# zser092/Focused-Attention-ViT

Measured on AMD Instinct MI355X. Metric: images/sec (train fwd+bwd) ViT-MHLA 224/p16, higher is better.
Workload: dtype bf16; 1 GPU; ViT-MHLA-Small (D384/12L/6H, window 7) 224x224 patch16, 197 tokens, 256 images/GPU; step = fwd + cross-entropy + bwd + grad all-reduce + AdamW; global_batch=256, parallelism=dp1, weights=random-init (seed 1234), hip_graph=False

## Files before the change

focused-attention-vit_amd/_abi.py:

```python
from __future__ import annotations

import ctypes as C
import os
import re

_HERE = os.path.dirname(os.path.abspath(__file__))
LIB_PATH = os.path.join(_HERE, "lib", "libfavit.so")
HEADER_PATH = os.path.join(os.path.dirname(_HERE), "include", "favit.h")

F32, BF16, FP8 = 0, 1, 2
F32X3 = 3
E4M3, E5M2 = 0, 1
ACT_NONE, ACT_GELU, ACT_DGELU, ACT_GELU_SAVEGRAD, ACT_MULAUX = 0, 1, 2, 3, 4
ERR_INVALID, ERR_UNSUPPORTED, ERR_ALIGN, ERR_LAUNCH = -1, -2, -3, -4
POOL = {"mean": 0, "max": 1, "attention": 2}

vp, i32, i64, u64, f32 = C.c_void_p, C.c_int32, C.c_int64, C.c_uint64, C.c_float


class GemmDesc(C.Structure):
    _fields_ = [
        ("A", vp), ("B", vp), ("C", vp), ("bias", vp), ("aux_in", vp), ("aux_out", vp), ("residual", vp),
        ("a_rowsum", vp),
        ("M", i64), ("N", i64), ("K", i64),
# ... 5 lines not shown
        ("scale_a", vp), ("scale_b", vp),
    ]


class SdpaDesc(C.Structure):
    _fields_ = [
        ("q", vp), ("k", vp), ("v", vp), ("o", vp), ("lse", vp), ("dout", vp), ("dq", vp), ("dk", vp), ("dv", vp),
        ("delta", vp), ("mask", vp), ("m_sb", i64), ("m_sq", i64),
        ("q_str", i64 * 3), ("k_str", i64 * 3), ("v_str", i64 * 3), ("o_str", i64 * 3), ("do_str", i64 * 3),
        ("dq_str", i64 * 3), ("dk_str", i64 * 3), ("dv_str", i64 * 3),
        ("B", i32), ("H", i32), ("Lq", i32), ("Lk", i32), ("hd", i32), ("dtype", i32),
        ("scale", f32), ("dropout_p", f32), ("seed", u64),
    ]


_SIGS = {
    "favit_abi_version": ([], C.c_int),
    "favit_strerror": ([C.c_int], C.c_char_p),
    "favit_set_dropout_epoch": ([vp], C.c_int),
    "favit_set_health_word": ([vp], C.c_int),
    "favit_gemm": ([C.POINTER(GemmDesc), vp], C.c_int),
    "favit_gemm_last_kernel": ([], C.c_char_p),
    "favit_ln_gemm": ([C.POINTER(GemmDesc), vp, i64, vp, vp, f32, vp, vp, vp, vp], C.c_int),
    "favit_gemm_grouped_tn": ([C.POINTER(GemmDesc), i32, vp], C.c_int),
    "favit_gemm_grouped_tn_workspace": ([C.POINTER(GemmDesc), i32], C.c_int64),
    "favit_gemm_grouped_tn_ws": ([C.POINTER(GemmDesc), i32, vp, i64, vp], C.c_int),
    "favit_gemm_grouped_last_splits": ([], C.c_int),
    "favit_cast": ([vp, C.c_int, vp, C.c_int, i64, vp], C.c_int),
    "favit_fp8_amax": ([vp, C.c_int, i64, i64, i64, vp, vp], C.c_int),
    "favit_fp8_quantize": ([vp, C.c_int, i64, i64, i64, vp, i64, vp, i64, C.c_int, vp, vp, vp, vp, vp, vp], C.c_int),
# ... 14 lines not shown
    "favit_mhla_attn_fwd": ([vp, vp, vp, i32, i32, i32, i32, i32, C.c_int, f32, u64, vp], C.c_int),
    "favit_mhla_attn_bwd": ([vp, vp, vp, vp, i32, i32, i32, i32, i32, C.c_int, f32, u64, vp], C.c_int),
    "favit_mhla_attn_lse_supported": ([i32, i32, i32, C.c_int], C.c_int),
    "favit_mhla_attn_fwd_lse": ([vp, vp, vp, vp, i32, i32, i32, i32, i32, C.c_int, f32, u64, vp], C.c_int),
    "favit_mhla_attn_bwd_lse": ([vp, vp, vp, vp, vp, vp, i32, i32, i32, i32, i32, C.c_int, f32, u64, vp], C.c_int),
    "favit_sdpa_fwd": ([C.POINTER(SdpaDesc), vp], C.c_int),
    "favit_sdpa_bwd": ([C.POINTER(SdpaDesc), vp], C.c_int),
    "favit_softmax_fwd": ([vp, vp, vp, C.c_int, vp, i64, i64, i32, i64, i32, i32, f32, u64, vp], C.c_int),
    "favit_softmax_bwd": ([vp, C.c_int, vp, vp, C.c_int, i64, i32, i32, f32, u64, vp], C.c_int),
    "favit_patchify_fwd": ([vp, vp, C.c_int, i32, i32, i32, i32, vp], C.c_int),
    "favit_patchify_bwd": ([vp, vp, i32, i32, i32, i32, vp], C.c_int),
    "favit_embed_prologue_fwd": ([vp, vp, vp, vp, i32, i32, i32, vp], C.c_int),
    "favit_embed_prologue_bwd": ([vp, vp, C.c_int, vp, vp, i32, i32, i32, vp], C.c_int),
    "favit_rows_cut_fwd": ([vp, vp, i32, i32, i32, i32, i32, vp], C.c_int),
    "favit_rows_cut_bwd": ([vp, vp, vp, C.c_int, i32, i32, i32, i32, i32, vp], C.c_int),
    "favit_dropout": ([vp, vp, C.c_int, i64, f32, u64, vp], C.c_int),
    "favit_sppp_map_patches": ([vp, vp, vp, vp, vp, vp, i32, i32, i32, vp], C.c_int),
    "favit_sppp_pool_fwd": ([vp, vp, vp, vp, vp, i32, i32, i32, i32, i32, vp], C.c_int),
    "favit_sppp_pool_bwd": ([vp, vp, vp, vp, vp, vp, vp, i32, i32, i32, i32, i32, vp], C.c_int),
    "favit_sppp_centroids": ([vp, vp, i32, i32, i32, vp], C.c_int),
    "favit_sppp_posenc_fwd": ([vp, vp, vp, i32, i32, i32, i32, vp], C.c_int),
    "favit_image_transform": ([vp, vp, vp, vp, vp, i32, i32, i32, i32, i32, i32, C.POINTER(f32), C.POINTER(f32), vp], C.c_int),
    "favit_image_transform_ragged": ([vp, vp, vp, vp, vp, vp, i32, i32, i32, i32, C.POINTER(f32), C.POINTER(f32), vp], C.c_int),
    "favit_slic_features_workspace": ([i32, i32, i32], C.c_int64),
    "favit_slic_features": ([vp, vp, i32, i32, i32, f32, i32, vp, vp], C.c_int),
    "favit_slic_cluster_workspace": ([i32, i32], C.c_int64),
    "favit_slic_cluster": ([vp, vp, vp, i32, i32, i32, i32, i32, i64, i32, vp, vp], C.c_int),
    "favit_slic_connect": ([vp, vp, vp, vp, vp, i32, i32, i32, i32, vp], C.c_int),
    "favit_cross_entropy": ([vp, vp, vp, vp, i32, i32, f32, vp], C.c_int),
    "favit_adamw": ([vp, vp, vp, vp, vp, i64, f32, f32, f32, f32, f32, f32, f32, f32, vp], C.c_int),
# ... 49 lines not shown
```

focused-attention-vit_amd/functional.py:

```python
from __future__ import annotations

import os
import weakref
from typing import List, Optional, Sequence, Tuple

import torch

from . import kernels as K
from ._abi import ACT_DGELU, ACT_GELU, ACT_GELU_SAVEGRAD, ACT_MULAUX, ACT_NONE

_STATE = {"cdt": torch.float32, "epoch": 0, "direct_grads": True, "grad_ready": None}


def set_direct_grads(on: bool) -> None:
    _STATE["direct_grads"] = bool(on)


def set_grad_ready_hook(fn) -> None:
    _STATE["grad_ready"] = fn


def _gt(p):
    if p is None or not _STATE["direct_grads"] or not getattr(p, "requires_grad", False):
        return None
# ... 546 lines not shown
        wp_c = wcast(wp)
        y = lin_fwd(o, wp_c, bp.detach(), M, D, D, torch.float32, residual=residual, drop=(pp, sp), site=wp)
        return y, (xn, weff, qkv, o, wp_c, mask, B, L, pa, sa, pp, sp, prm, lse)

    @staticmethod
    def out_dropout(saved):
        return saved[10], saved[11]

    def bwd(self, saved, dy_lp, premasked=False):
        xn, weff, qkv, o, wp_c, mask, B, L, pa, sa, pp, sp, prm, lse = saved
        wqkv, bqkv, wl, bl, wp, bp = prm
        M, D = xn.shape
        H, hd = self.H, D // self.H
        dym = K.dropout(dy_lp, pp, sp) if (pp > 0 and not premasked) else dy_lp
        do = lin_bwd_x(dym, wp_c, M, D, D, xn.dtype, site=wp)
        dwp, dbp = lin_bwd_w(dym, o, M, D, D, wp=wp, bp=bp)
        dqkv = K.mhla_attn_bwd(qkv, do, B, L, H, hd, self.W, mask, pa, sa, o=o if lse is not None else None, lse=lse)
        dxn = lin_bwd_x(dqkv, weff, M, 3 * D, D, xn.dtype, site=wqkv)
        dweff, dbeff = lin_bwd_w(dqkv, xn, M, 3 * D, D)
        tg = [_gt(p) for p in (wqkv, bqkv, wl, bl)]
        if all(t is not None for t in tg) and _DEFER["on"]:
            _DEFER["fold"].append((dweff, dbeff, wqkv.detach(), bqkv.detach(), wl.detach(), tg, H, (wqkv, bqkv, wl, bl)))
            return dxn, [None, None, None, None, dwp, dbp]
        if (_DEFER["on"] and not wqkv.requires_grad and not bqkv.requires_grad and tg[2] is not None and tg[3] is not None):
            _DEFER["fold"].append((dweff, dbeff, wqkv.detach(), bqkv.detach(), wl.detach(), [None, None, tg[2], tg[3]], H,
                                   (wl, bl)))
            return dxn, [None, None, None, None, dwp, dbp]
        flush_wgrads()
        if all(t is not None for t in tg):
            with _side_stream(dweff, dbeff):
                K.mhla_fold_bwd(dweff, dbeff, wqkv, bqkv, wl, H, out=tg)
                _ready(wqkv, bqkv, wl, bl)
            return dxn, [None, None, None, None, dwp, dbp]
        join_side_stream()
        dwqkv, dbqkv, dwl, dbl = K.mhla_fold_bwd(dweff, dbeff, wqkv, bqkv, wl, H)
        return dxn, [dwqkv, dbqkv, dwl, dbl, dwp, dbp]


class DenseChain:
    q8_fwd, q8_bwd = 0, 2
    """vit.MultiHeadAttention.forward (models/vit.py:77-104) and, with the
    nn.MultiheadAttention parameter names, the use_mhla=False branch
    (models/vit_mhla.py:57-62,96-101).  mask: key-keep [B,L] (torch MHA) or None."""

    def __init__(self, H, p_attn=0.0, p_proj=0.0, torch_mha=False):
        self.H, self.p_attn, self.p_proj, self.torch_mha = H, p_attn, p_proj, torch_mha
        self.names = (("in_proj_weight", "in_proj_bias", "out_proj.weight", "out_proj.bias") if torch_mha
                      else ("qkv.weight", "qkv.bias", "proj.weight", "proj.bias"))

    def _views(self, t, B, L, D, hd):
        ld = 3 * D
# ... 103 lines not shown
    def fwd(self, xn, prm, residual, training, ln=None):
        w1, b1, w2, b2 = prm
        M, D = xn.shape if ln is None else ln[0].shape
        Hd = w1.shape[0]
        Do = w2.shape[0]
        p = self.p if training else 0.0
        s1 = _seed() if p > 0 else 0
        s2 = _seed() if p > 0 else 0
        w1_c, w2_c = wcast(w1), wcast(w2)
        if ln is not None:
            sg = True
            h, pre, xn, mu, rs = lin_fwd_ln(ln[:3], w1_c, b1.detach(), M, Hd, D, get_compute_dtype(), act=ACT_GELU_SAVEGRAD,
                                            want_pre=True, drop=(p, s1))
            ln[3][:] = [xn, mu, rs]
        else:
            sg = xn.dtype != torch.float32
            h, pre = lin_fwd(xn, w1_c, b1.detach(), M, Hd, D, xn.dtype, act=ACT_GELU_SAVEGRAD if sg else ACT_GELU,
                             want_pre=True, drop=(p, s1), site=w1)
        y = lin_fwd(h, w2_c, b2.detach(), M, Do, Hd, torch.float32, residual=residual, drop=(p, s2), site=w2)
        return y, (xn, (pre, sg), h, w1_c, w2_c, p, s1, s2, prm)

    @staticmethod
    def out_dropout(saved):
        return saved[5], saved[7]

    def bwd(self, saved, dy_lp, premasked=False):
        xn, (pre, sg), h, w1_c, w2_c, p, s1, s2, prm = saved
        w1, b1, w2, b2 = prm
        M, D = xn.shape
        Hd, Do = w1_c.shape[0], w2_c.shape[0]
        dym = K.dropout(dy_lp, p, s2) if (p > 0 and not premasked) else dy_lp
        dpre = lin_bwd_x(dym, w2_c, M, Do, Hd, xn.dtype, dgelu_pre=pre, pre_is_grad=sg, drop=(p, s1), site=w2)
        dw2, db2 = lin_bwd_w(dym, h, M, Do, Hd, wp=w2, bp=b2)
        dxn = lin_bwd_x(dpre, w1_c, M, Hd, D, xn.dtype, site=w1)
        dw1, db1 = lin_bwd_w(dpre, xn, M, Hd, D, wp=w1, bp=b1)
        return dxn, [dw1, db1, dw2, db2]


class OpFn(torch.autograd.Function):

    @staticmethod
    def forward(ctx, op, n_in, *tensors):
        K.require_gpu(*[t for t in tensors if t is not None])
        ins, prm = tensors[:n_in], tensors[n_in:]
        out, saved = op.fwd(ins, prm)
        ctx.op, ctx.saved, ctx.n_in, ctx.n_prm = op, saved, n_in, len(prm)
        return out

    @staticmethod
    def backward(ctx, dout):
        din, dprm = ctx.op.bwd(ctx.saved, _as_f32(dout), ctx.needs_input_grad[2:2 + ctx.n_in])
# ... 122 lines not shown


def cls_only_cuts(specs: Sequence["BlockSpec"], L: int, mask, training: bool):
    if os.environ.get("FAVIT_NO_PRUNE") or mask is not None or not specs or _STATE.get("fp8"):
        return None
    if not all(isinstance(s.attn, MHLAChain) and isinstance(s.mlp, MLPChain) for s in specs):
        return None
    if len({s.attn.W for s in specs}) != 1:
        return None
    if training and any(s.attn.p_attn > 0 or s.attn.p_proj > 0 or s.mlp.p > 0 for s in specs):
        return None
    plan = cls_plan(L, specs[0].attn.W, len(specs))
    return plan if any(c is not None for c in plan) else None


class EncoderOp:

    def __init__(self, blocks: List[BlockSpec], mask=None, training=False, cuts=None):
        self.blocks, self.mask, self.training = blocks, mask, training
        self.cuts = list(cuts) if cuts is not None else None
        if self.cuts is not None and (len(self.cuts) != len(blocks) or mask is not None):
            raise ValueError("cuts: one entry per block, and no attention mask")

    def fwd(self, ins, prm):
        (x,) = ins
        B, L, D = x.shape
        M = B * L
        L_in = L
        cdt = get_compute_dtype()
        x = _as_f32(x).reshape(M, D)
        tapes = []
        fuse_ok = _LN_FUSE and cdt == torch.bfloat16 and get_compute_mode() == "bf16" and D % 64 == 0 and D <= 512
        pre = [None] * len(self.blocks)
        idx, fp, off = [], [], 0
        for bi, bs in enumerate(self.blocks):
            if isinstance(bs.attn, MHLAChain):
                idx.append(bi)
                fp.append(tuple(prm[off + 2:off + 6]))
            off += bs.n
        if 2 <= len(idx) <= 32 and len({(self.blocks[i].attn.H, tuple(q[0].shape)) for i, q in zip(idx, fp)}) == 1:
            for bi, we in zip(idx, K.mhla_fold_fwd_multi(fp, self.blocks[idx[0]].attn.H, cdt)):
                pre[bi] = we
        off = 0
        for bi, bs in enumerate(self.blocks):
            p = list(prm[off:off + bs.n])
            off += bs.n
            na = len(bs.attn.names)
            g1, b1 = p[0], p[1]
            pa = p[2:2 + na]
            g2, b2 = p[2 + na], p[3 + na]
            pm = p[4 + na:]
            cut = None
            if self.cuts is not None and self.cuts[bi] is not None and sum(self.cuts[bi]) < L:
                ca, cb = self.cuts[bi]
                x = K.rows_cut_fwd(x, B, L, ca, cb, D).reshape(B * (ca + cb), D)
                cut = (L, ca, cb)
                L = ca + cb
                M = B * L
            fuse = fuse_ok and M <= 16384
            if fuse and isinstance(bs.attn, (MHLAChain, DenseChain)):
                o1 = [None, None, None]
                kw = {"pre": pre[bi]} if pre[bi] is not None else {}
                x1, sa = bs.attn.fwd(None, pa, B, L, x, self.mask, self.training, ln=(x, g1.detach(), b1.detach(), o1), **kw)
                xn1, mu1, rs1 = o1
            else:
                xn1, mu1, rs1 = K.layernorm_fwd(x, D, g1, b1, M, D, cdt, q8=_q8_request(bs.attn, pa, "fwd", D))
                if pre[bi] is not None:
                    x1, sa = bs.attn.fwd(xn1, pa, B, L, x, self.mask, self.training, pre=pre[bi])
                else:
                    x1, sa = bs.attn.fwd(xn1, pa, B, L, x, self.mask, self.training)
            if fuse and isinstance(bs.mlp, MLPChain):
                o2 = [None, None, None]
                x2, sm = bs.mlp.fwd(None, pm, x1, self.training, ln=(x1, g2.detach(), b2.detach(), o2))
                xn2, mu2, rs2 = o2
            else:
                xn2, mu2, rs2 = K.layernorm_fwd(x1, D, g2, b2, M, D, cdt, q8=_q8_request(bs.mlp, pm, "fwd", D))
                x2, sm = bs.mlp.fwd(xn2, pm, x1, self.training)
            tapes.append((x, mu1, rs1, (g1, b1), sa, x1, mu2, rs2, (g2, b2), sm, (pa, pm), cut))
            x = x2
        return x.reshape(B, L, D), (tapes, B, L_in, D)

    def bwd(self, saved, dy, needs):
        tapes, B, L, D = saved
        g = dy.reshape(-1, D)
        g_lp = _as_cdt(g)
        grads = []
        begin_wgrads(per_block=any(tp[11] is not None for tp in tapes))
        begin_deferred()
        begin_zero_pool(sum(3 * D + 4 for bs in self.blocks if isinstance(bs.attn, MHLAChain)), dy.device)

        def ln_bwd(dxn, xin, gam, bet, mu, rs, dres, pd, q8=None, want_lp=True):
            M = xin.shape[0]
            if not gam.requires_grad and not bet.requires_grad:
                return K.layernorm_bwd(dxn, xin, D, gam, mu, rs, M, D, dres=dres, want_lp=want_lp, lp_drop=pd, frozen=True, q8=q8)
            tg_, tb_ = _gt(gam), _gt(bet)
            lst = _DEFER["ln"] if (_DEFER["on"] and tg_ is not None and tb_ is not None) else None
            n0 = len(lst) if lst is not None else 0
            out = K.layernorm_bwd(dxn, xin, D, gam, mu, rs, M, D, dres=dres, want_lp=want_lp, dg_out=tg_, db_out=tb_,
                                  lp_drop=pd, defer=lst, q8=q8)
            if lst is not None:
                lst[n0] = lst[n0] + ((gam, bet),)
            elif out[2] is None:
                _ready(gam, bet)
            return out
        try:
            order = list(zip(reversed(self.blocks), reversed(tapes)))
            premasked = False
            for bi, (bs, tp) in enumerate(order):
                x, mu1, rs1, (g1, b1), sa, x1, mu2, rs2, (g2, b2), sm, (pa_, _), cut = tp
                dxn2, gm = bs.mlp.bwd(sm, g_lp, premasked=premasked)
                pd = bs.attn.out_dropout(sa) if hasattr(bs.attn, "out_dropout") else (0.0, 0)
                g, g_lp, dg2, db2 = ln_bwd(dxn2, x1, g2, b2, mu2, rs2, g, pd,
                                           q8=_q8_request(bs.attn, pa_, "bwd", D) if hasattr(bs.attn, "out_dropout") else None)
                dxn1, ga = (bs.attn.bwd(sa, g_lp, premasked=pd[0] > 0) if hasattr(bs.attn, "out_dropout")
                            else bs.attn.bwd(sa, g_lp))
                pd = (0.0, 0)
                q8n = None
                if bi + 1 < len(order):
                    nbs, ntp = order[bi + 1]
                    pd = nbs.mlp.out_dropout(ntp[9])
                    q8n = _q8_request(nbs.mlp, ntp[10][1], "bwd", D)
                premasked = pd[0] > 0
                g, g_lp, dg1, db1 = ln_bwd(dxn1, x, g1, b1, mu1, rs1, g, pd, q8=q8n, want_lp=cut is None)
                if cut is not None:
                    n_in, ca, cb = cut
                    more = bi + 1 < len(order) and g.dtype != dxn1.dtype
                    g, g_lp = K.rows_cut_bwd(g, B, n_in, ca, cb, D, lp_dtype=dxn1.dtype if more else None)
                    g = g.reshape(B * n_in, D)
                    g_lp = g_lp.reshape(B * n_in, D) if g_lp is not None else g
                if flush_wgrads(force=False) and _STATE["grad_ready"] is not None:
                    flush_deferred()
                if not _SIDE["enabled"]:
                    join_side_stream()
                grads = [dg1, db1] + ga + [dg2, db2] + gm + grads
        except BaseException:
            _WG["list"] = None
            _SIDE["pending"].clear()
            _DEFER.update(on=False, fold=[], ln=[])
            end_zero_pool()
            raise
        end_wgrads()
        end_deferred()
# ... 153 lines not shown
```

focused-attention-vit_amd/kernels.py:

```python
from __future__ import annotations

import ctypes as C
from typing import Optional

import torch

from . import _abi
from ._abi import ACT_DGELU, ACT_GELU, ACT_NONE, BF16, F32, GemmDesc, SdpaDesc

_DT = {torch.float32: F32, torch.bfloat16: BF16}

_F32_GEMM = {"in_dtype": F32}


def set_f32_gemm_split(on: bool) -> None:
    _F32_GEMM["in_dtype"] = _abi.F32X3 if on else F32

GEMM_TRACE = None


def dt(t_or_dtype) -> int:
    d = t_or_dtype.dtype if torch.is_tensor(t_or_dtype) else t_or_dtype
    try:
        return _DT[d]
# ... 441 lines not shown
    return (out, None) if want_lse else out


def mhla_attn_bwd(qkv, dout, B, L, H, hd, W, mask=None, p=0.0, seed=0, o=None, lse=None):
    require_gpu(qkv, dout, mask, o, lse)
    dqkv = torch.empty_like(qkv)
    if o is not None and lse is not None:
        _abi.check(_abi.lib().favit_mhla_attn_bwd_lse(_p(qkv), _p(dout), _p(o), _p(lse), _p(dqkv), _p(mask), B, L, H, hd,
                                                      W, dt(qkv), p, seed, _st()), "favit_mhla_attn_bwd_lse")
        return dqkv
    _abi.check(_abi.lib().favit_mhla_attn_bwd(_p(qkv), _p(dout), _p(dqkv), _p(mask), B, L, H, hd, W, dt(qkv), p, seed,
                                              _st()), "favit_mhla_attn_bwd")
    return dqkv


def _sdpa_desc(q, k, v, o, lse, B, H, Lq, Lk, hd, scale, mask, m_sb, m_sq, p, seed):
    d = SdpaDesc()
    es = q.t.element_size()
    for name, vw in (("q", q), ("k", k), ("v", v), ("o", o)):
        setattr(d, name, vw.t.data_ptr() + vw.off * es)
        getattr(d, name + "_str")[:] = [vw.ld, vw.sb, vw.sh]
    d.lse = lse.data_ptr()
    d.mask = mask.data_ptr() if mask is not None else None
    d.m_sb, d.m_sq = m_sb, m_sq
    d.B, d.H, d.Lq, d.Lk, d.hd, d.dtype = B, H, Lq, Lk, hd, dt(q.t)
    d.scale, d.dropout_p, d.seed = scale, p, seed
    return d


def sdpa_fwd(q, k, v, o, B, H, Lq, Lk, hd, scale, mask=None, m_sb=0, m_sq=0, p=0.0, seed=0):
# ... 353 lines not shown
```

include/favit.h:

```cpp
#ifndef FAVIT_H_
#define FAVIT_H_

#include <stdint.h>

#ifdef __cplusplus
extern "C" {
#endif

#define FAVIT_ABI_VERSION 8
#define FAVIT_FP8_AMAX_SLOTS 256

enum { FAVIT_F32 = 0, FAVIT_BF16 = 1, FAVIT_FP8 = 2, FAVIT_F32X3 = 3 };
enum { FAVIT_E4M3 = 0, FAVIT_E5M2 = 1 };

enum {
  FAVIT_OK = 0,
  FAVIT_ERR_INVALID = -1,
  FAVIT_ERR_UNSUPPORTED = -2,
  FAVIT_ERR_ALIGN = -3,
  FAVIT_ERR_LAUNCH = -4
};

enum {
  FAVIT_ACT_NONE = 0,
// ... 152 lines not shown
int favit_sdpa_fwd(const favit_sdpa_t* s, void* stream);
int favit_sdpa_bwd(const favit_sdpa_t* s, void* stream);

int favit_patchify_fwd(const float* img, void* out, int out_dtype, int32_t B, int32_t C, int32_t HW, int32_t P,
                       void* stream);
int favit_patchify_bwd(const float* dpatch, float* dimg, int32_t B, int32_t C, int32_t HW, int32_t P, void* stream);
int favit_embed_prologue_fwd(const float* tok, const float* cls, const float* pos, float* x, int32_t B, int32_t N,
                             int32_t D, void* stream);
int favit_embed_prologue_bwd(const float* dx, void* dtok, int dtok_dtype, float* dcls, float* dpos, int32_t B,
                             int32_t N, int32_t D, void* stream);

int favit_rows_cut_fwd(const float* x, float* y, int32_t B, int32_t n_in, int32_t a, int32_t b, int32_t D, void* stream);
int favit_rows_cut_bwd(const float* dy, float* dx, void* dx_lp, int lp_dtype, int32_t B, int32_t n_in, int32_t a,
                       int32_t b, int32_t D, void* stream);

int favit_dropout(const void* x, void* y, int dtype, int64_t n, float p, uint64_t seed, void* stream);

int favit_sppp_map_patches(const int64_t* seg, int32_t* patch_rank, int32_t* n_tokens, int32_t* perm,
                           int32_t* offs, int64_t* dom_ws, int32_t B, int32_t HW, int32_t P, void* stream);
int favit_sppp_pool_fwd(const float* emb, const int32_t* perm, const int32_t* offs, float* out, int32_t* argmax,
                        int32_t kind, int32_t B, int32_t N, int32_t R, int32_t D, void* stream);
int favit_sppp_pool_bwd(const float* dout, const float* emb, const int32_t* patch_rank, const int32_t* perm,
                        const int32_t* offs, const int32_t* argmax, float* demb, int32_t kind, int32_t B,
                        int32_t N, int32_t R, int32_t D, void* stream);
int favit_sppp_centroids(const int64_t* seg, float* cent, int32_t B, int32_t HW, int32_t S, void* stream);
int favit_sppp_posenc_fwd(const float* x, const float* cent, float* y, int32_t B, int32_t L, int32_t D,
                          int32_t n_cent, void* stream);

int favit_cross_entropy(const float* logits, const int64_t* labels, float* loss_rows, float* dlogits, int32_t B,
                        int32_t C, float grad_scale, void* stream);
// ... 35 lines not shown
```

Before: 46700 images/sec.

## Add native C block forward/backward driver to cut Python dispatch per transformer block

Adds a C entry point that runs a whole MHLA transformer block forward (LN, QKV GEMM, attention, proj, LN, MLP) and its input-gradient backward chain in one host call, with activations stored in one preallocated tape buffer and backward scratch in one arena. The Python backward loop uses this path when no dropout, q8 or side-stream features are active, and computes weight gradients separately through factored-out helpers. This targets per-op Python and ctypes launch overhead and per-tensor allocations. In exchange it adds a second code path with strict geometry checks (head dim 64) and falls back to the old path otherwise.

Result: faster. 51370 images/sec (median of 6 runs) (+10.0%).

```diff
diff --git a/focused-attention-vit_amd/_abi.py b/focused-attention-vit_amd/_abi.py
--- a/focused-attention-vit_amd/_abi.py
+++ b/focused-attention-vit_amd/_abi.py
@@ -43,6 +43,18 @@
     ]
 
 
+class BlockDesc(C.Structure):
+    _fields_ = [
+        ("x", vp), ("tape", vp), ("g1", vp), ("b1", vp), ("g2", vp), ("b2", vp), ("weff", vp), ("beff", vp),
+        ("wproj", vp), ("bproj", vp), ("wfc1", vp), ("bfc1", vp), ("wfc2", vp), ("bfc2", vp),
+        ("tape_bytes", i64),
+        ("B", i32), ("n", i32), ("D", i32), ("H", i32), ("W", i32), ("hidden", i32), ("training", i32), ("eps", f32),
+    ]
+
+
+BLOCK_TAPE_SLOTS = ("xn1", "mu1", "rs1", "qkv", "o", "lse", "x1", "xn2", "mu2", "rs2", "h", "pre", "x2")
+BLOCK_BWD_SLOTS = ("dpre", "dxn2", "g1_f32", "g1_lp", "do", "dqkv", "dxn1", "g_out_f32", "g_out_lp", "part1", "part2")
+
 _SIGS = {
     "favit_abi_version": ([], C.c_int),
     "favit_strerror": ([C.c_int], C.c_char_p),
@@ -87,6 +99,10 @@
     "favit_embed_prologue_bwd": ([vp, vp, C.c_int, vp, vp, i32, i32, i32, vp], C.c_int),
     "favit_rows_cut_fwd": ([vp, vp, i32, i32, i32, i32, i32, vp], C.c_int),
     "favit_rows_cut_bwd": ([vp, vp, vp, C.c_int, i32, i32, i32, i32, i32, vp], C.c_int),
+    "favit_mhla_block_tape_layout": ([C.POINTER(BlockDesc), C.POINTER(i64)], C.c_int64),
+    "favit_mhla_block_bwd_layout": ([C.POINTER(BlockDesc), i32, C.POINTER(i64)], C.c_int64),
+    "favit_mhla_block_fwd": ([C.POINTER(BlockDesc), vp], C.c_int),
+    "favit_mhla_block_bwd": ([C.POINTER(BlockDesc), vp, vp, vp, i64, i32, vp], C.c_int),
     "favit_dropout": ([vp, vp, C.c_int, i64, f32, u64, vp], C.c_int),
     "favit_sppp_map_patches": ([vp, vp, vp, vp, vp, vp, i32, i32, i32, vp], C.c_int),
     "favit_sppp_pool_fwd": ([vp, vp, vp, vp, vp, i32, i32, i32, i32, i32, vp], C.c_int),
diff --git a/focused-attention-vit_amd/csrc/block.hip b/focused-attention-vit_amd/csrc/block.hip
--- /dev/null
+++ b/focused-attention-vit_amd/csrc/block.hip
@@ -0,0 +1,181 @@
+#include <string.h>
+
+#include "favit.h"
+
+namespace {
+constexpr int64_t ALIGN = 256;
+constexpr int TAPE_N = FAVIT_BLOCK_TAPE_SLOTS, BWD_N = FAVIT_BLOCK_BWD_SLOTS;
+enum { T_XN1, T_MU1, T_RS1, T_QKV, T_O, T_LSE, T_X1, T_XN2, T_MU2, T_RS2, T_H, T_PRE, T_X2 };
+enum { G_DPRE, G_DXN2, G_G1_F32, G_G1_LP, G_DO, G_DQKV, G_DXN1, G_OUT_F32, G_OUT_LP, G_PART1, G_PART2 };
+
+inline int64_t up(int64_t v) { return (v + ALIGN - 1) / ALIGN * ALIGN; }
+
+int check_geometry(const favit_mhla_block_t* d) {
+  if (!d) return FAVIT_ERR_INVALID;
+  if (d->B <= 0 || d->n <= 0 || d->D <= 0 || d->H <= 0 || d->W <= 0 || d->hidden <= 0 || !(d->eps > 0.f))
+    return FAVIT_ERR_INVALID;
+  if (d->D % 64 != 0 || d->D % d->H != 0 || d->D / d->H != 64) return FAVIT_ERR_UNSUPPORTED;
+  if (d->hidden % 8 != 0) return FAVIT_ERR_UNSUPPORTED;
+  if (!favit_mhla_attn_lse_supported(d->n, 64, d->W, FAVIT_BF16)) return FAVIT_ERR_UNSUPPORTED;
+  if ((int64_t)d->B * d->n >= (int64_t)1 << 31) return FAVIT_ERR_UNSUPPORTED;
+  return FAVIT_OK;
+}
+
+int64_t layout(const int64_t* sizes, int n, int64_t* offsets) {
+  int64_t off = 0;
+  for (int i = 0; i < n; ++i) {
+    if (offsets) offsets[i] = off;
+    off += up(sizes[i]);
+  }
+  return off;
+}
+
+void tape_sizes(const favit_mhla_block_t* d, int64_t* s) {
+  const int64_t M = (int64_t)d->B * d->n, D = d->D, Hd = d->hidden;
+  s[T_XN1] = M * D * 2; s[T_MU1] = M * 4; s[T_RS1] = M * 4;
+  s[T_QKV] = M * 3 * D * 2; s[T_O] = M * D * 2;
+  s[T_LSE] = d->training ? (int64_t)d->B * d->H * d->n * 4 : 0;
+  s[T_X1] = M * D * 4;
+  s[T_XN2] = M * D * 2; s[T_MU2] = M * 4; s[T_RS2] = M * 4;
+  s[T_H] = M * Hd * 2; s[T_PRE] = M * Hd * 2;
+  s[T_X2] = M * D * 4;
+}
+
+int32_t ln_parts(int64_t rows) { return (int32_t)((rows + 3) / 4 < 2048 ? (rows + 3) / 4 : 2048); }
+
+void bwd_sizes(const favit_mhla_block_t* d, int want_lp_out, int64_t* s) {
+  const int64_t M = (int64_t)d->B * d->n, D = d->D, Hd = d->hidden;
+  const int64_t part = 2 * (int64_t)ln_parts(M) * D * 4;
+  s[G_DPRE] = M * Hd * 2; s[G_DXN2] = M * D * 2;
+  s[G_G1_F32] = M * D * 4; s[G_G1_LP] = M * D * 2;
+  s[G_DO] = M * D * 2; s[G_DQKV] = M * 3 * D * 2; s[G_DXN1] = M * D * 2;
+  s[G_OUT_F32] = M * D * 4; s[G_OUT_LP] = want_lp_out ? M * D * 2 : 0;
+  s[G_PART1] = part; s[G_PART2] = part;
+}
+
+favit_gemm_t gemm_base(const void* A, const void* B, void* C, int64_t M, int64_t N, int64_t K, int64_t ldb, int b_kmajor,
+                       int out_dtype) {
+  favit_gemm_t g;
+  memset(&g, 0, sizeof(g));
+  g.A = A; g.B = B; g.C = C;
+  g.M = M; g.N = N; g.K = K;
+  g.lda = K; g.ldb = ldb; g.ldc = N;
+  g.batch = 1; g.batch_inner = 1;
+  g.a_kmajor = 1; g.b_kmajor = b_kmajor;
+  g.in_dtype = FAVIT_BF16; g.out_dtype = out_dtype;
+  g.act = FAVIT_ACT_NONE;
+  g.alpha = 1.0f;
+  return g;
+}
+
+int check_params(const favit_mhla_block_t* d) {
+  if (!d->x || !d->tape || !d->g1 || !d->b1 || !d->g2 || !d->b2 || !d->weff || !d->beff || !d->wproj || !d->bproj ||
+      !d->wfc1 || !d->bfc1 || !d->wfc2 || !d->bfc2)
+    return FAVIT_ERR_INVALID;
+  if (((uintptr_t)d->tape % ALIGN) != 0 || ((uintptr_t)d->x % 16) != 0) return FAVIT_ERR_ALIGN;
+  return FAVIT_OK;
+}
+}
+
+extern "C" int64_t favit_mhla_block_tape_layout(const favit_mhla_block_t* desc, int64_t* offsets_out) {
+  const int rc = check_geometry(desc);
+  if (rc != FAVIT_OK) return rc;
+  int64_t s[TAPE_N];
+  tape_sizes(desc, s);
+  return layout(s, TAPE_N, offsets_out);
+}
+
+extern "C" int64_t favit_mhla_block_bwd_layout(const favit_mhla_block_t* desc, int32_t want_lp_out, int64_t* offsets_out) {
+  const int rc = check_geometry(desc);
+  if (rc != FAVIT_OK) return rc;
+  int64_t s[BWD_N];
+  bwd_sizes(desc, want_lp_out, s);
+  return layout(s, BWD_N, offsets_out);
+}
+
+extern "C" int favit_mhla_block_fwd(const favit_mhla_block_t* d, void* stream) {
+  int rc = check_geometry(d);
+  if (rc != FAVIT_OK) return rc;
+  if ((rc = check_params(d)) != FAVIT_OK) return rc;
+  int64_t s[TAPE_N], o[TAPE_N];
+  tape_sizes(d, s);
+  if (d->tape_bytes < layout(s, TAPE_N, o)) return FAVIT_ERR_INVALID;
+  char* t = reinterpret_cast<char*>(d->tape);
+  const int64_t M = (int64_t)d->B * d->n;
+  const int32_t D = d->D, Hd = d->hidden;
+  float* x1 = reinterpret_cast<float*>(t + o[T_X1]);
+  if ((rc = favit_layernorm_fwd(d->x, D, d->g1, d->b1, t + o[T_XN1], FAVIT_BF16, reinterpret_cast<float*>(t + o[T_MU1]),
+                                reinterpret_cast<float*>(t + o[T_RS1]), M, D, d->eps, stream)) != FAVIT_OK)
+    return rc;
+  favit_gemm_t g = gemm_base(t + o[T_XN1], d->weff, t + o[T_QKV], M, 3 * D, D, D, 1, FAVIT_BF16);
+  g.bias = d->beff;
+  g.ld_aux_out = 3 * D; g.ld_res = 3 * D;
+  if ((rc = favit_gemm(&g, stream)) != FAVIT_OK) return rc;
+  rc = d->training ? favit_mhla_attn_fwd_lse(t + o[T_QKV], t + o[T_O], reinterpret_cast<float*>(t + o[T_LSE]), nullptr,
+                                             d->B, d->n, d->H, 64, d->W, FAVIT_BF16, 0.f, 0, stream)
+                   : favit_mhla_attn_fwd(t + o[T_QKV], t + o[T_O], nullptr, d->B, d->n, d->H, 64, d->W, FAVIT_BF16, 0.f, 0,
+                                         stream);
+  if (rc != FAVIT_OK) return rc;
+  g = gemm_base(t + o[T_O], d->wproj, x1, M, D, D, D, 1, FAVIT_F32);
+  g.bias = d->bproj; g.residual = d->x;
+  g.ld_aux_out = D; g.ld_res = D;
+  if ((rc = favit_gemm(&g, stream)) != FAVIT_OK) return rc;
+  if ((rc = favit_layernorm_fwd(x1, D, d->g2, d->b2, t + o[T_XN2], FAVIT_BF16, reinterpret_cast<float*>(t + o[T_MU2]),
+                                reinterpret_cast<float*>(t + o[T_RS2]), M, D, d->eps, stream)) != FAVIT_OK)
+    return rc;
+  g = gemm_base(t + o[T_XN2], d->wfc1, t + o[T_H], M, Hd, D, D, 1, FAVIT_BF16);
+  g.bias = d->bfc1; g.act = FAVIT_ACT_GELU_SAVEGRAD; g.aux_out = t + o[T_PRE];
+  g.ld_aux_out = Hd; g.ld_res = Hd;
+  if ((rc = favit_gemm(&g, stream)) != FAVIT_OK) return rc;
+  g = gemm_base(t + o[T_H], d->wfc2, t + o[T_X2], M, D, Hd, Hd, 1, FAVIT_F32);
+  g.bias = d->bfc2; g.residual = x1;
+  g.ld_aux_out = D; g.ld_res = D;
+  return favit_gemm(&g, stream);
+}
+
+extern "C" int favit_mhla_block_bwd(const favit_mhla_block_t* d, const float* g_f32, const void* g_lp, void* bwd_buffers,
+                                    int64_t bwd_bytes, int32_t want_lp_out, void* stream) {
+  int rc = check_geometry(d);
+  if (rc != FAVIT_OK) return rc;
+  if ((rc = check_params(d)) != FAVIT_OK) return rc;
+  if (!d->training || !g_f32 || !g_lp || !bwd_buffers) return FAVIT_ERR_INVALID;
+  if (((uintptr_t)bwd_buffers % ALIGN) != 0 || ((uintptr_t)g_f32 % 16) != 0 || ((uintptr_t)g_lp % 16) != 0)
+    return FAVIT_ERR_ALIGN;
+  int64_t s[TAPE_N], o[TAPE_N], bs[BWD_N], b[BWD_N];
+  tape_sizes(d, s);
+  if (d->tape_bytes < layout(s, TAPE_N, o)) return FAVIT_ERR_INVALID;
+  bwd_sizes(d, want_lp_out, bs);
+  if (bwd_bytes < layout(bs, BWD_N, b)) return FAVIT_ERR_INVALID;
+  char* t = reinterpret_cast<char*>(d->tape);
+  char* w = reinterpret_cast<char*>(bwd_buffers);
+  const int64_t M = (int64_t)d->B * d->n;
+  const int32_t D = d->D, Hd = d->hidden, np = ln_parts(M);
+  float* g1 = reinterpret_cast<float*>(w + b[G_G1_F32]);
+  float* part1 = reinterpret_cast<float*>(w + b[G_PART1]);
+  float* part2 = reinterpret_cast<float*>(w + b[G_PART2]);
+  favit_gemm_t g = gemm_base(g_lp, d->wfc2, w + b[G_DPRE], M, Hd, D, Hd, 0, FAVIT_BF16);
+  g.act = FAVIT_ACT_MULAUX; g.aux_in = t + o[T_PRE]; g.ld_aux_in = Hd;
+  if ((rc = favit_gemm(&g, stream)) != FAVIT_OK) return rc;
+  g = gemm_base(w + b[G_DPRE], d->wfc1, w + b[G_DXN2], M, D, Hd, D, 0, FAVIT_BF16);
+  g.ld_aux_in = D;
+  if ((rc = favit_gemm(&g, stream)) != FAVIT_OK) return rc;
+  if ((rc = favit_layernorm_bwd(w + b[G_DXN2], FAVIT_BF16, reinterpret_cast<const float*>(t + o[T_X1]), D, d->g2,
+                                reinterpret_cast<const float*>(t + o[T_MU2]), reinterpret_cast<const float*>(t + o[T_RS2]),
+                                g_f32, g1, D, w + b[G_G1_LP], FAVIT_BF16, part2, part2 + (int64_t)np * D, np, nullptr,
+                                nullptr, 1, M, D, 0.f, 0, stream)) != FAVIT_OK)
+    return rc;
+  g = gemm_base(w + b[G_G1_LP], d->wproj, w + b[G_DO], M, D, D, D, 0, FAVIT_BF16);
+  g.ld_aux_in = D;
+  if ((rc = favit_gemm(&g, stream)) != FAVIT_OK) return rc;
+  if ((rc = favit_mhla_attn_bwd_lse(t + o[T_QKV], w + b[G_DO], t + o[T_O], reinterpret_cast<const float*>(t + o[T_LSE]),
+                                    w + b[G_DQKV], nullptr, d->B, d->n, d->H, 64, d->W, FAVIT_BF16, 0.f, 0, stream)) !=
+      FAVIT_OK)
+    return rc;
+  g = gemm_base(w + b[G_DQKV], d->weff, w + b[G_DXN1], M, D, 3 * D, D, 0, FAVIT_BF16);
+  g.ld_aux_in = D;
+  if ((rc = favit_gemm(&g, stream)) != FAVIT_OK) return rc;
+  return favit_layernorm_bwd(w + b[G_DXN1], FAVIT_BF16, d->x, D, d->g1, reinterpret_cast<const float*>(t + o[T_MU1]),
+                             reinterpret_cast<const float*>(t + o[T_RS1]), g1, reinterpret_cast<float*>(w + b[G_OUT_F32]), D,
+                             want_lp_out ? w + b[G_OUT_LP] : nullptr, FAVIT_BF16, part1, part1 + (int64_t)np * D, np, nullptr,
+                             nullptr, 1, M, D, 0.f, 0, stream);
+}
diff --git a/focused-attention-vit_amd/functional.py b/focused-attention-vit_amd/functional.py
--- a/focused-attention-vit_amd/functional.py
+++ b/focused-attention-vit_amd/functional.py
@@ -584,27 +584,37 @@
         H, hd = self.H, D // self.H
         dym = K.dropout(dy_lp, pp, sp) if (pp > 0 and not premasked) else dy_lp
         do = lin_bwd_x(dym, wp_c, M, D, D, xn.dtype, site=wp)
-        dwp, dbp = lin_bwd_w(dym, o, M, D, D, wp=wp, bp=bp)
+        dwp, dbp = self.proj_grads(dym, o, prm)
         dqkv = K.mhla_attn_bwd(qkv, do, B, L, H, hd, self.W, mask, pa, sa, o=o if lse is not None else None, lse=lse)
         dxn = lin_bwd_x(dqkv, weff, M, 3 * D, D, xn.dtype, site=wqkv)
+        return dxn, self.qkv_grads(dqkv, xn, prm) + [dwp, dbp]
+
+    @staticmethod
+    def proj_grads(dym, o, prm):
+        M, D = o.shape
+        return lin_bwd_w(dym, o, M, D, D, wp=prm[4], bp=prm[5])
+
+    def qkv_grads(self, dqkv, xn, prm):
+        wqkv, bqkv, wl, bl = prm[:4]
+        M, D = xn.shape
+        H = self.H
         dweff, dbeff = lin_bwd_w(dqkv, xn, M, 3 * D, D)
         tg = [_gt(p) for p in (wqkv, bqkv, wl, bl)]
         if all(t is not None for t in tg) and _DEFER["on"]:
             _DEFER["fold"].append((dweff, dbeff, wqkv.detach(), bqkv.detach(), wl.detach(), tg, H, (wqkv, bqkv, wl, bl)))
-            return dxn, [None, None, None, None, dwp, dbp]
+            return [None, None, None, None]
         if (_DEFER["on"] and not wqkv.requires_grad and not bqkv.requires_grad and tg[2] is not None and tg[3] is not None):
             _DEFER["fold"].append((dweff, dbeff, wqkv.detach(), bqkv.detach(), wl.detach(), [None, None, tg[2], tg[3]], H,
                                    (wl, bl)))
-            return dxn, [None, None, None, None, dwp, dbp]
+            return [None, None, None, None]
         flush_wgrads()
         if all(t is not None for t in tg):
             with _side_stream(dweff, dbeff):
                 K.mhla_fold_bwd(dweff, dbeff, wqkv, bqkv, wl, H, out=tg)
                 _ready(wqkv, bqkv, wl, bl)
-            return dxn, [None, None, None, None, dwp, dbp]
+            return [None, None, None, None]
         join_side_stream()
-        dwqkv, dbqkv, dwl, dbl = K.mhla_fold_bwd(dweff, dbeff, wqkv, bqkv, wl, H)
-        return dxn, [dwqkv, dbqkv, dwl, dbl, dwp, dbp]
+        return list(K.mhla_fold_bwd(dweff, dbeff, wqkv, bqkv, wl, H))
 
 
 class DenseChain:
@@ -738,11 +748,15 @@
                                             want_pre=True, drop=(p, s1))
             ln[3][:] = [xn, mu, rs]
         else:
-            sg = xn.dtype != torch.float32
+            sg = self.saves_gelu_grad(xn.dtype)
             h, pre = lin_fwd(xn, w1_c, b1.detach(), M, Hd, D, xn.dtype, act=ACT_GELU_SAVEGRAD if sg else ACT_GELU,
                              want_pre=True, drop=(p, s1), site=w1)
         y = lin_fwd(h, w2_c, b2.detach(), M, Do, Hd, torch.float32, residual=residual, drop=(p, s2), site=w2)
         return y, (xn, (pre, sg), h, w1_c, w2_c, p, s1, s2, prm)
+
+    @staticmethod
+    def saves_gelu_grad(cdt) -> bool:
+        return cdt != torch.float32
 
     @staticmethod
     def out_dropout(saved):
@@ -755,10 +769,18 @@
         Hd, Do = w1_c.shape[0], w2_c.shape[0]
         dym = K.dropout(dy_lp, p, s2) if (p > 0 and not premasked) else dy_lp
         dpre = lin_bwd_x(dym, w2_c, M, Do, Hd, xn.dtype, dgelu_pre=pre, pre_is_grad=sg, drop=(p, s1), site=w2)
-        dw2, db2 = lin_bwd_w(dym, h, M, Do, Hd, wp=w2, bp=b2)
+        dw2, db2 = self.fc2_grads(dym, h, prm)
         dxn = lin_bwd_x(dpre, w1_c, M, Hd, D, xn.dtype, site=w1)
-        dw1, db1 = lin_bwd_w(dpre, xn, M, Hd, D, wp=w1, bp=b1)
+        dw1, db1 = self.fc1_grads(dpre, xn, prm)
         return dxn, [dw1, db1, dw2, db2]
+
+    @staticmethod
+    def fc2_grads(dym, h, prm):
+        return lin_bwd_w(dym, h, dym.shape[0], dym.shape[1], h.shape[1], wp=prm[2], bp=prm[3])
+
+    @staticmethod
+    def fc1_grads(dpre, xn, prm):
+        return lin_bwd_w(dpre, xn, dpre.shape[0], dpre.shape[1], xn.shape[1], wp=prm[0], bp=prm[1])
 
 
 class OpFn(torch.autograd.Function):
@@ -911,6 +933,61 @@
     return plan if any(c is not None for c in plan) else None
 
 
+_NATIVE = {"on": True}
+
+
+def set_native_blocks(on: bool) -> None:
+    _NATIVE["on"] = bool(on)
+
+
+def _native_blocks_on() -> bool:
+    return (_NATIVE["on"] and K.GEMM_TRACE is None and not _SIDE["enabled"] and not _LN_FUSE
+            and get_compute_mode() == "bf16" and not os.environ.get("FAVIT_NO_NATIVE_BLOCKS"))
+
+
+def _carve(flat, off, shape):
+    st, n = [], 1
+    for d in reversed(shape):
+        st.append(n)
+        n *= d
+    return torch.as_strided(flat, shape, tuple(reversed(st)), off)
+
+
+class _NativeTape:
+    __slots__ = ("plan", "buf", "x", "ln", "pa", "pm", "weff", "wc", "cut", "_bf", "_f32")
+
+    def __init__(self, plan, buf, x, ln, pa, pm, weff, wc, cut):
+        self.plan, self.buf, self.x, self.ln, self.pa, self.pm, self.weff, self.wc, self.cut = \
+            plan, buf, x, ln, pa, pm, weff, wc, cut
+        self._bf = self._f32 = None
+
+    def bf(self, name, *shape):
+        if self._bf is None:
+            self._bf = self.buf.view(torch.bfloat16)
+        return _carve(self._bf, self.plan.off[name][0] // 2, shape)
+
+    def f32(self, name, *shape):
+        if self._f32 is None:
+            self._f32 = self.buf.view(torch.float32)
+        return _carve(self._f32, self.plan.off[name][0] // 4, shape)
+
+    def unpack(self):
+        pl = self.plan
+        M, D, Hd = pl.M, pl.D, pl.hidden
+        (g1, b1, g2, b2), (wp_c, w1_c, w2_c) = self.ln, self.wc
+        lse = self.f32("lse", pl.B, pl.H, pl.n) if pl.off["lse"][1] else None
+        sa = (self.bf("xn1", M, D), self.weff, self.bf("qkv", M, 3 * D), self.bf("o", M, D), wp_c, None, pl.B, pl.n,
+              0.0, 0, 0.0, 0, self.pa, lse)
+        sm = (self.bf("xn2", M, D), (self.bf("pre", M, Hd), MLPChain.saves_gelu_grad(torch.bfloat16)), self.bf("h", M, Hd),
+              w1_c, w2_c, 0.0, 0, 0, self.pm)
+        return (self.x, self.f32("mu1", M), self.f32("rs1", M), (g1, b1), sa, self.f32("x1", M, D), self.f32("mu2", M),
+                self.f32("rs2", M), (g2, b2), sm, (self.pa, self.pm), self.cut)
+
+
+def _tape_cut(tp):
+    return tp.cut if isinstance(tp, _NativeTape) else tp[11]
+
+
 class EncoderOp:
 
     def __init__(self, blocks: List[BlockSpec], mask=None, training=False, cuts=None):
@@ -938,6 +1015,7 @@
         if 2 <= len(idx) <= 32 and len({(self.blocks[i].attn.H, tuple(q[0].shape)) for i, q in zip(idx, fp)}) == 1:
             for bi, we in zip(idx, K.mhla_fold_fwd_multi(fp, self.blocks[idx[0]].attn.H, cdt)):
                 pre[bi] = we
+        native = self.mask is None and x.is_cuda and _native_blocks_on()
         off = 0
         for bi, bs in enumerate(self.blocks):
             p = list(prm[off:off + bs.n])
@@ -954,6 +1032,12 @@
                 cut = (L, ca, cb)
                 L = ca + cb
                 M = B * L
+            if native and pre[bi] is not None:
+                nt = self._fwd_native(bs, p, x, B, L, D, pre[bi], cut)
+                if nt is not None:
+                    tapes.append(nt)
+                    x = nt.f32("x2", M, D)
+                    continue
             fuse = fuse_ok and M <= 16384
             if fuse and isinstance(bs.attn, (MHLAChain, DenseChain)):
                 o1 = [None, None, None]
@@ -977,12 +1061,71 @@
             x = x2
         return x.reshape(B, L, D), (tapes, B, L_in, D)
 
+    def _fwd_native(self, bs, p, x, B, L, D, pre, cut):
+        at, ml = bs.attn, bs.mlp
+        if not (isinstance(at, MHLAChain) and isinstance(ml, MLPChain)) or len(p) != 14:
+            return None
+        if self.training and (at.p_attn > 0 or at.p_proj > 0 or ml.p > 0):
+            return None
+        g1, b1, wqkv, bqkv, wl, bl, wp, bp, g2, b2, w1, c1, w2, c2 = p
+        Hd = w1.shape[0]
+        if tuple(w2.shape) != (D, Hd) or tuple(w1.shape) != (Hd, D) or tuple(wp.shape) != (D, D):
+            return None
+        if any(t.dtype != torch.float32 or not t.is_contiguous() for t in (g1, b1, g2, b2, bp, c1, c2)):
+            return None
+        weff, beff = pre
+        wc = (wcast(wp), wcast(w1), wcast(w2))
+        if weff.dtype != torch.bfloat16 or any(w.dtype != torch.bfloat16 or not w.is_contiguous() for w in wc):
+            return None
+        plans = getattr(g1, "_favit_blocks", None)
+        if plans is None:
+            plans = g1._favit_blocks = {}
+        key = (B, L, D, at.H, at.W, Hd, bool(self.training))
+        if key not in plans:
+            plans[key] = K.mhla_block_plan(*key)
+        plan = plans[key]
+        if plan is None:
+            return None
+        buf = torch.empty(plan.tape_bytes, dtype=torch.uint8, device=x.device)
+        if K.mhla_block_fwd(plan, x, buf, g1, b1, g2, b2, weff, beff, wc[0], bp, wc[1], c1, wc[2], c2) != 0:
+            return None
+        return _NativeTape(plan, buf, x, (g1, b1, g2, b2), p[2:8], p[10:], weff, wc, cut)
+
+    def _bwd_native(self, bs, tp, g, g_lp):
+        plan = tp.plan
+        g1, b1, g2, b2 = tp.ln
+        tg = [_gt(q) for q in tp.ln]
+        if any(t is None for t in tg):
+            return None
+        M, D, Hd = plan.M, plan.D, plan.hidden
+        if (g.dtype != torch.float32 or g_lp.dtype != torch.bfloat16 or tuple(g.shape) != (M, D) or not g.is_contiguous()
+                or tuple(g_lp.shape) != (M, D) or not g_lp.is_contiguous()):
+            return None
+        want_lp = tp.cut is None
+        arena = torch.empty(plan.bwd_bytes[want_lp], dtype=torch.uint8, device=g.device)
+        wp_c, w1_c, w2_c = tp.wc
+        if K.mhla_block_bwd(plan, tp.x, tp.buf, g1, g2, tp.weff, wp_c, w1_c, w2_c, g, g_lp, arena, want_lp) != 0:
+            return None
+        bo = plan.boff[want_lp]
+        abf, af = arena.view(torch.bfloat16), arena.view(torch.float32)
+        part = lambda k: _carve(af, bo[k][0] // 4, (2, plan.nparts, D))
+        g1_lp = _carve(abf, bo["g1_lp"][0] // 2, (M, D))
+        dqkv = _carve(abf, bo["dqkv"][0] // 2, (M, 3 * D))
+        dw2, db2 = bs.mlp.fc2_grads(g_lp, tp.bf("h", M, Hd), tp.pm)
+        dw1, db1 = bs.mlp.fc1_grads(_carve(abf, bo["dpre"][0] // 2, (M, Hd)), tp.bf("xn2", M, D), tp.pm)
+        _DEFER["ln"].append((part("part2"), tg[2], tg[3], (g2, b2)))
+        dwp, dbp = bs.attn.proj_grads(g1_lp, tp.bf("o", M, D), tp.pa)
+        ga = bs.attn.qkv_grads(dqkv, tp.bf("xn1", M, D), tp.pa) + [dwp, dbp]
+        _DEFER["ln"].append((part("part1"), tg[0], tg[1], (g1, b1)))
+        g_out = _carve(af, bo["g_out_f32"][0] // 4, (M, D))
+        return g_out, (_carve(abf, bo["g_out_lp"][0] // 2, (M, D)) if want_lp else None), ga, [dw1, db1, dw2, db2]
+
     def bwd(self, saved, dy, needs):
         tapes, B, L, D = saved
         g = dy.reshape(-1, D)
         g_lp = _as_cdt(g)
         grads = []
-        begin_wgrads(per_block=any(tp[11] is not None for tp in tapes))
+        begin_wgrads(per_block=any(_tape_cut(tp) is not None for tp in tapes))
         begin_deferred()
         begin_zero_pool(sum(3 * D + 4 for bs in self.blocks if isinstance(bs.attn, MHLAChain)), dy.device)
 
@@ -1004,25 +1147,36 @@
             order = list(zip(reversed(self.blocks), reversed(tapes)))
             premasked = False
             for bi, (bs, tp) in enumerate(order):
-                x, mu1, rs1, (g1, b1), sa, x1, mu2, rs2, (g2, b2), sm, (pa_, _), cut = tp
-                dxn2, gm = bs.mlp.bwd(sm, g_lp, premasked=premasked)
-                pd = bs.attn.out_dropout(sa) if hasattr(bs.attn, "out_dropout") else (0.0, 0)
-                g, g_lp, dg2, db2 = ln_bwd(dxn2, x1, g2, b2, mu2, rs2, g, pd,
-                                           q8=_q8_request(bs.attn, pa_, "bwd", D) if hasattr(bs.attn, "out_dropout") else None)
-                dxn1, ga = (bs.attn.bwd(sa, g_lp, premasked=pd[0] > 0) if hasattr(bs.attn, "out_dropout")
-                            else bs.attn.bwd(sa, g_lp))
-                pd = (0.0, 0)
-                q8n = None
-                if bi + 1 < len(order):
+                pd_n, q8n = (0.0, 0), None
+                if bi + 1 < len(order) and not isinstance(order[bi + 1][1], _NativeTape):
                     nbs, ntp = order[bi + 1]
-                    pd = nbs.mlp.out_dropout(ntp[9])
+                    pd_n = nbs.mlp.out_dropout(ntp[9])
                     q8n = _q8_request(nbs.mlp, ntp[10][1], "bwd", D)
-                premasked = pd[0] > 0
-                g, g_lp, dg1, db1 = ln_bwd(dxn1, x, g1, b1, mu1, rs1, g, pd, q8=q8n, want_lp=cut is None)
+                done = None
+                if isinstance(tp, _NativeTape):
+                    if not premasked and pd_n[0] == 0 and q8n is None and _DEFER["on"] and _native_blocks_on():
+                        done = self._bwd_native(bs, tp, g, g_lp)
+                    if done is None:
+                        tp = tp.unpack()
+                if done is not None:
+                    g, g_lp, ga, gm = done
+                    dg1 = db1 = dg2 = db2 = None
+                    cut, lp_dt = tp.cut, torch.bfloat16
+                else:
+                    x, mu1, rs1, (g1, b1), sa, x1, mu2, rs2, (g2, b2), sm, (pa_, _), cut = tp
+                    dxn2, gm = bs.mlp.bwd(sm, g_lp, premasked=premasked)
+                    pd = bs.attn.out_dropout(sa) if hasattr(bs.attn, "out_dropout") else (0.0, 0)
+                    g, g_lp, dg2, db2 = ln_bwd(dxn2, x1, g2, b2, mu2, rs2, g, pd,
+                                               q8=_q8_request(bs.attn, pa_, "bwd", D) if hasattr(bs.attn, "out_dropout") else None)
+                    dxn1, ga = (bs.attn.bwd(sa, g_lp, premasked=pd[0] > 0) if hasattr(bs.attn, "out_dropout")
+                                else bs.attn.bwd(sa, g_lp))
+                    g, g_lp, dg1, db1 = ln_bwd(dxn1, x, g1, b1, mu1, rs1, g, pd_n, q8=q8n, want_lp=cut is None)
+                    lp_dt = dxn1.dtype
+                premasked = pd_n[0] > 0
                 if cut is not None:
                     n_in, ca, cb = cut
-                    more = bi + 1 < len(order) and g.dtype != dxn1.dtype
-                    g, g_lp = K.rows_cut_bwd(g, B, n_in, ca, cb, D, lp_dtype=dxn1.dtype if more else None)
+                    more = bi + 1 < len(order) and g.dtype != lp_dt
+                    g, g_lp = K.rows_cut_bwd(g, B, n_in, ca, cb, D, lp_dtype=lp_dt if more else None)
                     g = g.reshape(B * n_in, D)
                     g_lp = g_lp.reshape(B * n_in, D) if g_lp is not None else g
                 if flush_wgrads(force=False) and _STATE["grad_ready"] is not None:
diff --git a/focused-attention-vit_amd/kernels.py b/focused-attention-vit_amd/kernels.py
--- a/focused-attention-vit_amd/kernels.py
+++ b/focused-attention-vit_amd/kernels.py
@@ -479,6 +479,59 @@
     return dqkv
 
 
+class BlockPlan:
+    __slots__ = ("desc", "ref", "M", "D", "hidden", "B", "n", "H", "nparts", "tape_bytes", "off", "bwd_bytes", "boff")
+
+
+def mhla_block_plan(B, n, D, H, W, hidden, training, eps=1e-5) -> Optional[BlockPlan]:
+    d = _abi.BlockDesc()
+    d.B, d.n, d.D, d.H, d.W, d.hidden, d.training, d.eps = B, n, D, H, W, hidden, int(bool(training)), eps
+    lib = _abi.lib()
+    to = (C.c_int64 * len(_abi.BLOCK_TAPE_SLOTS))()
+    tape_bytes = lib.favit_mhla_block_tape_layout(C.byref(d), to)
+    if tape_bytes < 0:
+        return None
+    p = BlockPlan()
+    p.desc, p.ref, p.M, p.D, p.hidden, p.B, p.n, p.H = d, C.byref(d), B * n, D, hidden, B, n, H
+    p.nparts = int(min(2048, (B * n + 3) // 4))
+    p.tape_bytes = d.tape_bytes = tape_bytes
+    ends = list(to[1:]) + [tape_bytes]
+    p.off = {k: (to[i], ends[i] - to[i]) for i, k in enumerate(_abi.BLOCK_TAPE_SLOTS)}
+    p.bwd_bytes, p.boff = [], []
+    for want_lp in (0, 1):
+        bo = (C.c_int64 * len(_abi.BLOCK_BWD_SLOTS))()
+        nb = lib.favit_mhla_block_bwd_layout(C.byref(d), want_lp, bo)
+        ends = list(bo[1:]) + [nb]
+        p.bwd_bytes.append(nb)
+        p.boff.append({k: (bo[i], ends[i] - bo[i]) for i, k in enumerate(_abi.BLOCK_BWD_SLOTS)})
+    return p
+
+
+def _block_code(code: int, what: str) -> int:
+    if code == _abi.ERR_LAUNCH:
+        _abi.check(code, what)
+    return code
+
+
+def mhla_block_fwd(plan: BlockPlan, x, tape, g1, b1, g2, b2, weff, beff, wproj, bproj, wfc1, bfc1, wfc2, bfc2) -> int:
+    d = plan.desc
+    d.x, d.tape, d.tape_bytes = x.data_ptr(), tape.data_ptr(), tape.numel()
+    d.g1, d.b1, d.g2, d.b2 = g1.data_ptr(), b1.data_ptr(), g2.data_ptr(), b2.data_ptr()
+    d.weff, d.beff, d.wproj, d.bproj = weff.data_ptr(), beff.data_ptr(), wproj.data_ptr(), bproj.data_ptr()
+    d.wfc1, d.bfc1, d.wfc2, d.bfc2 = wfc1.data_ptr(), bfc1.data_ptr(), wfc2.data_ptr(), bfc2.data_ptr()
+    return _block_code(_abi.lib().favit_mhla_block_fwd(plan.ref, _st()), "favit_mhla_block_fwd")
+
+
+def mhla_block_bwd(plan: BlockPlan, x, tape, g1, g2, weff, wproj, wfc1, wfc2, g, g_lp, arena, want_lp_out: bool) -> int:
+    d = plan.desc
+    d.x, d.tape, d.tape_bytes = x.data_ptr(), tape.data_ptr(), tape.numel()
+    d.g1, d.g2 = g1.data_ptr(), g2.data_ptr()
+    d.weff, d.wproj, d.wfc1, d.wfc2 = weff.data_ptr(), wproj.data_ptr(), wfc1.data_ptr(), wfc2.data_ptr()
+    return _block_code(_abi.lib().favit_mhla_block_bwd(plan.ref, g.data_ptr(), g_lp.data_ptr(), arena.data_ptr(),
+                                                       arena.numel(), int(bool(want_lp_out)), _st()),
+                       "favit_mhla_block_bwd")
+
+
 def _sdpa_desc(q, k, v, o, lse, B, H, Lq, Lk, hd, scale, mask, m_sb, m_sq, p, seed):
     d = SdpaDesc()
     es = q.t.element_size()
diff --git a/include/favit.h b/include/favit.h
--- a/include/favit.h
+++ b/include/favit.h
@@ -190,6 +190,35 @@
 int favit_rows_cut_bwd(const float* dy, float* dx, void* dx_lp, int lp_dtype, int32_t B, int32_t n_in, int32_t a,
                        int32_t b, int32_t D, void* stream);
 
+#define FAVIT_BLOCK_TAPE_SLOTS 13
+#define FAVIT_BLOCK_BWD_SLOTS 11
+typedef struct favit_mhla_block {
+  const float* x;
+  void* tape;
+  const float* g1;
+  const float* b1;
+  const float* g2;
+  const float* b2;
+  const void* weff;
+  const float* beff;
+  const void* wproj;
+  const float* bproj;
+  const void* wfc1;
+  const float* bfc1;
+  const void* wfc2;
+  const float* bfc2;
+  int64_t tape_bytes;
+  int32_t B, n, D, H, W, hidden;
+  int32_t training;
+  float eps;
+} favit_mhla_block_t;
+int64_t favit_mhla_block_tape_layout(const favit_mhla_block_t* desc, int64_t* offsets_out );
+int64_t favit_mhla_block_bwd_layout(const favit_mhla_block_t* desc, int32_t want_lp_out,
+                                    int64_t* offsets_out );
+int favit_mhla_block_fwd(const favit_mhla_block_t* desc, void* stream);
+int favit_mhla_block_bwd(const favit_mhla_block_t* desc, const float* g_f32, const void* g_lp, void* bwd_buffers,
+                         int64_t bwd_bytes, int32_t want_lp_out, void* stream);
+
 int favit_dropout(const void* x, void* y, int dtype, int64_t n, float p, uint64_t seed, void* stream);
 
 int favit_sppp_map_patches(const int64_t* seg, int32_t* patch_rank, int32_t* n_tokens, int32_t* perm,
```
